# ChaitIITB/ReplicatingGPT

Measured on AMD Instinct MI355X. Metric: train tokens/sec at 1/2/4/8 MI355X + MFMA util, char-GPT block 256, higher is better.
Workload: dtype bf16; 1 GPU; c2: char-GPT 6L/6H/384d, block 256, batch 64/GPU, dropout 0.2, AdamW, full train step; global_batch=64, seq_len=256, parallelism=dp1, world_size=1, graph=True

## Files before the change

include/charpt.h:

```cpp
#ifndef CHARPT_H
#define CHARPT_H
#include <stdint.h>

#ifdef __cplusplus
extern "C" {
#endif

enum { CG_OK = 0, CG_EINVAL = 1, CG_EHIP = 2, CG_EUNSUPPORTED = 3 };
enum { CG_F32 = 0, CG_BF16 = 1 };
enum { CG_BITS = 2 };

enum {
    CG_EPI_STORE = 0,
    CG_EPI_BIAS = 1,
    CG_EPI_BIAS_RELU = 2,
    CG_EPI_BIAS_RESID = 3,
    CG_EPI_BIAS_DROP_RESID = 4,
    CG_EPI_RELU_BWD = 5,
    CG_EPI_STORE_ROWDOT = 7
};

typedef struct {
    int kind;
    const float* bias;
    const float* resid;
    int64_t ld_resid;
    const void* aux;
    int aux_dtype;
    int64_t ld_aux;
    double dropout_p;
    uint64_t seed;
    const uint64_t* rng_call;
    int site;
    float beta;
    float* colpart;
    int flags;
} cg_epilogue_t;

enum { CG_GEMM_SLAB_BF16 = 1, CG_GEMM_DEFER_REDUCE = 2 };
enum { CG_DEFER = 1 };

const char* cg_last_error_string(void);
int cg_version(void);
int cg_set_tuning(const char* key, int value);
int cg_device_info(int* n_cu, int* arch_major, int* arch_minor);
int cg_timing_event_create(void** event);
int cg_timing_event_record(void* event, void* stream);
int cg_timing_event_elapsed(void* start, void* end, float* ms);
int cg_timing_event_destroy(void* event);

int cg_counter_add(int64_t* counter, int64_t delta, void* stream);
int cg_rng_snapshot(uint64_t* counter, uint64_t* snap, void* stream);
int cg_dropout_mask(float* dst, int64_t n, double p, uint64_t seed, const uint64_t* rng_call, int site,
                    void* stream);
int cg_dropout_apply(const float* x, int64_t rows, int64_t C, int64_t ldx, void* y, int y_dtype, double p,
                     uint64_t seed, const uint64_t* rng_call, int site, void* stream);
int cg_sum_f32(const float* x, int64_t n, float scale, float* out, float* ws, void* stream);
int cg_cast_f32_bf16(const float* x, uint16_t* y, int64_t n, void* stream);

int cg_gather_batch(const void* data, int data_is_u8, const int64_t* ix, int64_t* x, int64_t* y,
                    int64_t B, int64_t T, void* stream);

int cg_gather_pairs(const int64_t* table, const int64_t* plen, const int64_t* tlen, const int64_t* ix, int64_t* x,
                    int64_t* y, int64_t B, int64_t T, int64_t pad_token, int64_t ignore_index, void* stream);

int cg_embed_fwd(const int64_t* idx, const float* wte, const float* wpe, float* x, int64_t B, int64_t T,
                 int64_t C, int64_t V, void* stream);
int64_t cg_embed_bwd_workspace(int64_t B, int64_t T, int64_t C, int64_t V);
int cg_embed_bwd(const int64_t* idx, const float* dx, float* dwte, float* dwpe, int64_t B, int64_t T,
                 int64_t C, int64_t V, int accumulate, void* workspace, void* stream);

int cg_layernorm_fwd(const float* x, const float* w, const float* b, void* y, int y_dtype, float* mean,
                     float* rstd, int64_t rows, int64_t C, float eps, void* stream);
int64_t cg_layernorm_bwd_workspace(int64_t rows, int64_t C);
int cg_layernorm_bwd(const void* dy, int dy_dtype, const float* x, const float* w, const float* mean,
                     const float* rstd, const float* dres, float* dx, uint16_t* dx_bf16, float* dw, float* db,
                     int accumulate, void* workspace, int64_t rows, int64_t C, void* stream);
int cg_layernorm_bwd_ex(const void* dy, int dy_dtype, const float* x, const float* w, const float* mean,
                        const float* rstd, const float* dres, float* dx, uint16_t* lp_out, double lp_dropout_p,
                        uint64_t lp_seed, const uint64_t* lp_rng_call, int lp_site, float* dw, float* db,
                        float* lp_colsum, int accumulate, int colsum_accumulate, void* workspace, int64_t rows,
                        int64_t C, void* stream);
int cg_layernorm_bwd_rows(const void* dy, int dy_dtype, const float* x, const float* w, const float* mean,
                          const float* rstd, const float* dres, float* dx, uint16_t* lp_out, double lp_dropout_p,
                          uint64_t lp_seed, const uint64_t* lp_rng_call, int lp_site, int lp_colsum,
                          void* workspace, int64_t rows, int64_t C, void* stream);
int cg_layernorm_bwd_reduce(const void* workspace, int64_t rows, int64_t C, int lp_colsum_partials, float* dw,
                            float* db, float* lp_colsum, int accumulate, int colsum_accumulate, void* stream);
int cg_layernorm_bwd_reduce_ex(const void* workspace, int64_t rows, int64_t C, int lp_colsum_partials, float* dw,
                               float* db, float* lp_colsum, int accumulate, int colsum_accumulate, int flags,
                               void* stream);

int64_t cg_gemm_workspace(int64_t M, int64_t N, int split_k);
int cg_gemm_colpart_supported(int a_trans, int b_trans, int64_t M, int64_t N, int64_t K, int64_t lda, int64_t ldb,
                              int64_t ldc);
int cg_gemm_relu_bits_supported(int a_trans, int b_trans, int64_t M, int64_t N, int64_t K, int64_t lda, int64_t ldb,
                                int64_t ldc);
// ... 145 lines not shown
```

replicatinggpt_amd/_lib.py:

```python
import ctypes
import os
import re

import torch

_HERE = os.path.dirname(os.path.abspath(__file__))
LIB_PATH = os.environ.get("CHARPT_LIB") or os.path.join(_HERE, "libcharpt_hip.so")
HEADER_PATH = os.path.join(os.path.dirname(_HERE), "include", "charpt.h")

CG_F32, CG_BF16, CG_BITS = 0, 1, 2
EPI_STORE, EPI_BIAS, EPI_BIAS_RELU, EPI_BIAS_RESID, EPI_BIAS_DROP_RESID, EPI_RELU_BWD = range(6)
EPI_STORE_ROWDOT = 7
GEMM_SLAB_BF16, GEMM_DEFER_REDUCE = 1, 2
DEFER = 1

c_i64, c_int, c_dbl, c_flt, c_u64, P = ctypes.c_int64, ctypes.c_int, ctypes.c_double, ctypes.c_float, ctypes.c_uint64, ctypes.c_void_p


class Epilogue(ctypes.Structure):
    _fields_ = [("kind", c_int), ("bias", P), ("resid", P), ("ld_resid", c_i64), ("aux", P), ("aux_dtype", c_int),
                ("ld_aux", c_i64), ("dropout_p", c_dbl), ("seed", c_u64), ("rng_call", P), ("site", c_int),
                ("beta", c_flt), ("colpart", P), ("flags", c_int)]


class WgradProblem(ctypes.Structure):
    _fields_ = [("M", c_i64), ("N", c_i64), ("K", c_i64), ("A", P), ("lda", c_i64), ("B", P), ("ldb", c_i64), ("C", P),
                ("ldc", c_i64), ("beta", c_flt), ("split_k", c_int), ("workspace", P), ("flags", c_int)]


_SIGS = {
    "cg_last_error_string": (ctypes.c_char_p, []),
    "cg_version": (c_int, []),
    "cg_set_tuning": (c_int, [ctypes.c_char_p, c_int]),
    "cg_device_info": (c_int, [P, P, P]),
    "cg_counter_add": (c_int, [P, c_i64, P]),
    "cg_rng_snapshot": (c_int, [P, P, P]),
    "cg_dropout_mask": (c_int, [P, c_i64, c_dbl, c_u64, P, c_int, P]),
    "cg_dropout_apply": (c_int, [P, c_i64, c_i64, c_i64, P, c_int, c_dbl, c_u64, P, c_int, P]),
    "cg_sum_f32": (c_int, [P, c_i64, c_flt, P, P, P]),
    "cg_cast_f32_bf16": (c_int, [P, P, c_i64, P]),
    "cg_gather_batch": (c_int, [P, c_int, P, P, P, c_i64, c_i64, P]),
    "cg_gather_pairs": (c_int, [P, P, P, P, P, P, c_i64, c_i64, c_i64, c_i64, P]),
    "cg_embed_fwd": (c_int, [P, P, P, P, c_i64, c_i64, c_i64, c_i64, P]),
    "cg_embed_bwd_workspace": (c_i64, [c_i64, c_i64, c_i64, c_i64]),
    "cg_embed_bwd": (c_int, [P, P, P, P, c_i64, c_i64, c_i64, c_i64, c_int, P, P]),
    "cg_layernorm_fwd": (c_int, [P, P, P, P, c_int, P, P, c_i64, c_i64, c_flt, P]),
    "cg_layernorm_bwd_workspace": (c_i64, [c_i64, c_i64]),
    "cg_layernorm_bwd": (c_int, [P, c_int, P, P, P, P, P, P, P, P, P, c_int, P, c_i64, c_i64, P]),
    "cg_layernorm_bwd_ex": (c_int, [P, c_int, P, P, P, P, P, P, P, c_dbl, c_u64, P, c_int, P, P, P, c_int, c_int, P,
                                    c_i64, c_i64, P]),
    "cg_layernorm_bwd_rows": (c_int, [P, c_int, P, P, P, P, P, P, P, c_dbl, c_u64, P, c_int, c_int, P, c_i64, c_i64,
                                      P]),
    "cg_layernorm_bwd_reduce": (c_int, [P, c_i64, c_i64, c_int, P, P, P, c_int, c_int, P]),
    "cg_layernorm_bwd_reduce_ex": (c_int, [P, c_i64, c_i64, c_int, P, P, P, c_int, c_int, c_int, P]),
    "cg_gemm_workspace": (c_i64, [c_i64, c_i64, c_int]),
    "cg_gemm_colpart_supported": (c_int, [c_int, c_int, c_i64, c_i64, c_i64, c_i64, c_i64, c_i64]),
    "cg_gemm_relu_bits_supported": (c_int, [c_int, c_int, c_i64, c_i64, c_i64, c_i64, c_i64, c_i64]),
    "cg_gemm_rowdot_supported": (c_int, [c_int, c_int, c_i64, c_i64, c_i64, c_i64, c_i64, c_i64]),
    "cg_linear_rows_f32_supported": (c_int, [c_i64, c_i64, c_i64]),
    "cg_decode_qkv_f32": (c_int, [c_i64, c_i64, c_i64, P, c_i64, P, P, c_flt, P, c_i64, P, c_i64, P, c_i64, P, P, P]),
    "cg_linear_rows_f32": (c_int, [c_i64, c_i64, c_i64, P, c_i64, P, P, c_flt, P, c_i64, P, c_int, P, c_i64, P, c_i64, P]),
    "cg_ffn_fwd_f32_supported": (c_int, [c_i64, c_i64, c_i64]),
    "cg_ffn_fwd_f32": (c_int, [c_i64, c_i64, c_i64, P, c_i64, P, P, c_flt, P, c_i64, P, P, c_i64, P, P, c_i64, P,
                               c_i64, P]),
    "cg_gemm_resid_layernorm_supported": (c_int, [c_i64, c_i64, c_i64]),
    "cg_gemm_resid_layernorm": (c_int, [c_i64, c_i64, c_i64, P, c_i64, P, c_i64, P, c_i64, ctypes.POINTER(Epilogue), P, P,
                                        P, P, P, c_flt, P]),
    "cg_flush_deferred": (c_int, [P]),
    "cg_discard_deferred": (c_int, [P, P]),
    "cg_reduce_rows": (c_int, [P, c_i64, c_i64, P, c_int, P]),
    "cg_reduce_rows_ex": (c_int, [P, c_i64, c_i64, P, c_int, c_int, P]),
    "cg_gemm": (c_int, [c_int, c_int, c_int, c_i64, c_i64, c_i64, P, c_i64, P, c_i64, P, c_int, c_i64,
                        ctypes.POINTER(Epilogue), c_int, P, P]),
    "cg_gemm_wgrad_group_supported": (c_int, [ctypes.POINTER(WgradProblem), c_int]),
    "cg_gemm_wgrad_group": (c_int, [ctypes.POINTER(WgradProblem), c_int, P]),
    "cg_colsum_workspace": (c_i64, [c_i64, c_i64]),
    "cg_colsum": (c_int, [P, c_int, c_i64, c_i64, c_i64, P, c_int, P, P]),
    "cg_attn_fwd": (c_int, [c_int, c_i64, c_i64, c_i64, c_i64, P, P, P, c_i64, P, c_i64, P, c_flt, c_dbl, c_u64, P,
                            c_int, P, P]),
    "cg_attn_fwd_premasked": (c_int, [c_int, c_i64, c_i64, c_i64, c_i64, P, P, P, c_i64, P, c_i64, P, c_flt, c_dbl,
                                      c_u64, P, c_int, P, P]),
    "cg_attn_dropmask": (c_int, [c_i64, c_i64, c_i64, c_dbl, c_u64, P, c_int, P, P]),
    "cg_layernorm_fwd_attn_dropmask": (c_int, [P, P, P, P, c_int, P, P, c_i64, c_i64, c_flt, c_i64, c_i64, c_i64,
                                               c_dbl, c_u64, P, c_int, P, P]),
    "cg_attn_mask_bytes": (c_i64, [c_i64, c_i64, c_i64]),
    "cg_attn_bwd_workspace": (c_i64, [c_i64, c_i64, c_i64, c_i64]),
    "cg_attn_bwd": (c_int, [c_int, c_i64, c_i64, c_i64, c_i64, P, P, P, c_i64, P, c_i64, P, c_i64, P, P, P, P, c_i64,
                            c_flt, c_dbl, c_u64, P, c_int, P, P, P]),
    "cg_attn_bwd_delta": (c_int, [c_int, c_i64, c_i64, c_i64, c_i64, P, P, P, c_i64, P, c_i64, P, c_i64, P, P, P, P,
                                  P, c_i64, c_flt, c_dbl, c_u64, P, c_int, P, P, P]),
    "cg_ce_fwd": (c_int, [P, c_i64, c_i64, c_i64, P, P, P, P]),
    "cg_ce_bwd": (c_int, [P, c_i64, c_i64, c_i64, P, P, P, c_flt, P, c_i64, P, P]),
    "cg_head_workspace": (c_i64, [c_i64, c_i64]),
    "cg_head_fwd": (c_int, [P, P, c_i64, P, P, P, P, P, P, c_i64, c_i64, c_i64, P]),
    "cg_head_bwd": (c_int, [P, P, P, P, c_flt, P, P, c_i64, P, c_int, P, c_i64, c_i64, P]),
    "cg_head_bwd_ex": (c_int, [P, P, P, P, c_flt, P, P, c_i64, P, c_int, P, c_i64, c_i64, c_int, P]),
    "cg_head_masked_workspace": (c_i64, [c_i64, c_i64]),
    "cg_head_fwd_masked": (c_int, [P, P, c_i64, P, P, c_i64, P, P, P, P, P, c_i64, c_i64, c_i64, P]),
    "cg_head_bwd_masked": (c_int, [P, P, P, c_i64, P, P, P, P, c_i64, P, c_int, P, c_i64, c_i64, c_int, P]),
    "cg_ce_fwd_masked": (c_int, [P, c_i64, c_i64, P, c_i64, P, P, P]),
    "cg_ce_mean_masked_workspace": (c_i64, [c_i64]),
    "cg_ce_mean_masked": (c_int, [P, P, c_i64, c_i64, P, P, P, P]),
    "cg_ce_bwd_masked": (c_int, [P, c_i64, c_i64, P, c_i64, P, P, P, P, P, P]),
    "cg_decode_window": (c_int, [P, c_i64, c_i64, c_i64, P, P, P]),
    "cg_decode_embed": (c_int, [P, c_i64, P, P, c_i64, P, P, c_i64, P]),
    "cg_decode_kv_append": (c_int, [P, c_i64, c_i64, c_i64, c_i64, c_i64, c_i64, c_i64, P, P, P, P]),
    "cg_decode_attn": (c_int, [P, c_i64, P, P, c_i64, c_i64, c_i64, c_i64, c_i64, c_i64, P, c_i64, c_flt, P, c_i64,
                               P]),
    "cg_decode_sample": (c_int, [P, c_i64, c_i64, c_i64, c_int, P, P, P, c_i64, P]),
    "cg_decode_sample_filtered": (c_int, [P, c_i64, c_i64, c_i64, P, P, P, P, c_i64, P]),
# ... 71 lines not shown
```

replicatinggpt_amd/csrc/gemm.hip:

```cpp
#include "defer.h"

using namespace cg;

namespace {

constexpr int GBM = 64, GBN = 64, GBK = 16;

template <typename TA, typename TB, typename TC>
__global__ __launch_bounds__(256) void k_gemm_generic(int a_trans, int b_trans, int64_t M, int64_t N, int64_t K,
                                                      const TA* __restrict__ A, int64_t lda,
                                                      const TB* __restrict__ B, int64_t ldb, TC* __restrict__ C,
                                                      int64_t ldc, EpiArgs epi, int split_k, int64_t kchunk,
                                                      float* __restrict__ ws) {
    __shared__ float As[GBK][GBM + 4];
    __shared__ float Bs[GBK][GBN + 4];
    const int tid = threadIdx.x, lane = tid & 63, wave = tid >> 6;
    const int wm = wave >> 1, wn = wave & 1;
    const int64_t tilesN = (N + GBN - 1) / GBN;
    const int64_t m0 = (int64_t)(blockIdx.x / tilesN) * GBM;
    const int64_t n0 = (int64_t)(blockIdx.x % tilesN) * GBN;
    const int split = blockIdx.y;
    const int64_t kb = split * kchunk;
    const int64_t ke = kb + kchunk < K ? kb + kchunk : K;

// ... 78 lines not shown
    a.ld_resid = e->ld_resid;
    a.aux = e->aux;
    a.aux_dtype = e->aux_dtype;
    a.ld_aux = e->ld_aux;
    a.thr = e->dropout_p > 0 ? dropout_threshold(e->dropout_p) : 0u;
    a.dscale = e->dropout_p > 0 ? dropout_scale(e->dropout_p) : 1.f;
    a.seed = e->seed;
    a.rng_call = e->rng_call;
    a.site = e->site;
    a.beta = e->beta;
    a.colpart = e->colpart;
    return a;
}

template <typename TA, typename TB>
int launch_generic(int a_trans, int b_trans, int64_t M, int64_t N, int64_t K, const void* A, int64_t lda,
                   const void* B, int64_t ldb, void* C, int c_dtype, int64_t ldc, const EpiArgs& e, int split_k,
                   void* ws, hipStream_t st) {
    int64_t kchunk = (K + split_k - 1) / split_k;
    kchunk = (kchunk + GBK - 1) / GBK * GBK;
    const int64_t tiles = ((M + GBM - 1) / GBM) * ((N + GBN - 1) / GBN);
    dim3 grid((unsigned)tiles, (unsigned)split_k);
    if (c_dtype == CG_BF16)
        k_gemm_generic<TA, TB, bf16_t><<<grid, 256, 0, st>>>(a_trans, b_trans, M, N, K, (const TA*)A, lda,
                                                             (const TB*)B, ldb, (bf16_t*)C, ldc, e, split_k, kchunk,
                                                             (float*)ws);
    else
        k_gemm_generic<TA, TB, float><<<grid, 256, 0, st>>>(a_trans, b_trans, M, N, K, (const TA*)A, lda,
                                                            (const TB*)B, ldb, (float*)C, ldc, e, split_k, kchunk,
                                                            (float*)ws);
    return CG_OK;
}

}

namespace cg {
int g_gemm_variant = 0;
int g_gemm_max_grid = 0;
int g_gemm_group_p8 = 0;
int g_gemm_group_pk = 0;
int g_gemm_n96 = 1;
}

extern "C" int cg_gemm_colpart_supported(int a_trans, int b_trans, int64_t M, int64_t N, int64_t K, int64_t lda,
                                         int64_t ldb, int64_t ldc) {
    return gemm_colpart_supported(a_trans, b_trans, M, N, K, lda, ldb, ldc) ? 1 : 0;
}

extern "C" int cg_gemm_relu_bits_supported(int a_trans, int b_trans, int64_t M, int64_t N, int64_t K, int64_t lda,
                                           int64_t ldb, int64_t ldc) {
    return gemm_relu_bits_supported(a_trans, b_trans, M, N, K, lda, ldb, ldc) ? 1 : 0;
}

extern "C" int cg_gemm_rowdot_supported(int a_trans, int b_trans, int64_t M, int64_t N, int64_t K, int64_t lda,
                                        int64_t ldb, int64_t ldc) {
    return gemm_rowdot_supported(a_trans, b_trans, M, N, K, lda, ldb, ldc) ? 1 : 0;
}

extern "C" int64_t cg_gemm_workspace(int64_t M, int64_t N, int split_k) {
    return split_k > 1 ? (int64_t)split_k * M * N * (int64_t)sizeof(float) : 0;
}

extern "C" int cg_gemm_resid_layernorm_supported(int64_t M, int64_t N, int64_t K) {
    return gemm_resid_ln_supported(M, N, K) ? 1 : 0;
}

extern "C" int cg_gemm_resid_layernorm(int64_t M, int64_t N, int64_t K, const void* A, int64_t lda, const void* W,
                                       int64_t ldw, float* out, int64_t ldc, const cg_epilogue_t* epi,
                                       const float* ln_w, const float* ln_b, void* y, float* mean, float* rstd,
                                       float eps, void* stream) {
    CG_REQUIRE(gemm_resid_ln_supported(M, N, K),
               "cg_gemm_resid_layernorm: unsupported shape M=%lld N=%lld K=%lld (N == 384, M %% 64 == 0, K %% 64 == 0)",
               (long long)M, (long long)N, (long long)K);
    CG_REQUIRE(epi && (epi->kind == CG_EPI_BIAS_RESID || epi->kind == CG_EPI_BIAS_DROP_RESID) && epi->bias &&
                   epi->resid && epi->beta == 0.f && epi->flags == 0 && !epi->colpart,
               "cg_gemm_resid_layernorm: needs a BIAS_RESID / BIAS_DROP_RESID epilogue with bias and residual, beta 0");
    CG_REQUIRE(A && W && out && ln_w && ln_b && y && mean && rstd, "cg_gemm_resid_layernorm: null pointer");
    CG_REQUIRE(lda >= K && ldw >= K && lda % 8 == 0 && ldw % 8 == 0 && ldc >= N && ldc % 4 == 0 &&
                   epi->ld_resid >= N && epi->ld_resid % 4 == 0,
               "cg_gemm_resid_layernorm: bad leading dimensions");
    CG_REQUIRE((((uintptr_t)A | (uintptr_t)W | (uintptr_t)out | (uintptr_t)epi->resid | (uintptr_t)epi->bias |
                 (uintptr_t)ln_w | (uintptr_t)ln_b | (uintptr_t)y) & 15) == 0,
               "cg_gemm_resid_layernorm: operands must be 16-B aligned");
    const EpiArgs e = make_epi(epi);
    gemm_resid_ln_launch(M, K, (const bf16_t*)A, lda, (const bf16_t*)W, ldw, out, ldc, e, ln_w, ln_b, (bf16_t*)y, mean,
                         rstd, eps, (hipStream_t)stream);
    CG_LAUNCH_CHECK("cg_gemm_resid_layernorm");
    return CG_OK;
}

extern "C" int cg_gemm(int op_dtype, int a_trans, int b_trans, int64_t M, int64_t N, int64_t K, const void* A,
                       int64_t lda, const void* B, int64_t ldb, void* C, int c_dtype, int64_t ldc,
                       const cg_epilogue_t* epi, int split_k, void* workspace, void* stream) {
    CG_REQUIRE(M > 0 && N > 0 && K > 0, "cg_gemm: empty problem M=%lld N=%lld K=%lld", (long long)M, (long long)N,
               (long long)K);
    CG_REQUIRE(split_k >= 1 && split_k <= 64, "cg_gemm: split_k out of range");
    CG_REQUIRE(split_k == 1 || workspace, "cg_gemm: split_k > 1 needs a workspace");
    CG_REQUIRE(op_dtype == CG_BF16 || op_dtype == CG_F32, "cg_gemm: bad op dtype");
    hipStream_t st = (hipStream_t)stream;
    EpiArgs e = make_epi(epi);
    CG_REQUIRE(split_k == 1 || e.kind == CG_EPI_STORE || e.kind == CG_EPI_BIAS || e.kind == CG_EPI_BIAS_RESID,
               "cg_gemm: split-K supports STORE/BIAS/BIAS_RESID epilogues only");
    const bool vec4 = N % 4 == 0 && ldc % 4 == 0 && M * N < (int64_t)1 << 31 &&
                      (((uintptr_t)C | (uintptr_t)workspace | (uintptr_t)(e.bias ? e.bias : (const float*)C) |
                        (uintptr_t)(e.resid ? e.resid : (const float*)C)) & 15) == 0 &&
                      (!e.resid || e.ld_resid % 4 == 0);
// ... 131 lines not shown
```

replicatinggpt_amd/csrc/gemm_bf16.hip:

```cpp
#include "gemm_tile.h"

namespace cg {
namespace {
using namespace gt;

template <bool TR, int R, int THREADS>
struct Operand {
    static constexpr int BYTES = R * FBK * 2;
    static constexpr int NCH = BYTES / (THREADS * 16);
    static_assert(NCH >= 1 && NCH * THREADS * 16 == BYTES, "tile/thread mismatch");
    struct Stage {
        uint4 v[NCH];
    };
    static __device__ __forceinline__ Stage load(const bf16_t* __restrict__ X, int64_t ld, int64_t r0, int64_t k0,
                                                 int tid) {
        Stage s;
#pragma unroll
        for (int i = 0; i < NCH; ++i) {
            const int lin = tid + i * THREADS;
            if (!TR) {
                const int r = lin >> 3, c = lin & 7;
                s.v[i] = *(const uint4*)(X + (r0 + r) * ld + k0 + c * 8);
            } else {
                constexpr int CPR = R / 8;
// ... 140 lines not shown
        v = (!at && split_k == 1 && M % 256 == 0 && N % 256 == 0 && t256 >= 2 * (int64_t)gemm_cu_count()) ? 24 : 9;
    }
    return v;
}

static bool fast_shape_ok(int64_t M, int64_t N, int64_t K, int64_t lda, int64_t ldb, int64_t ldc, int split_k) {
    return N % 128 == 0 && K % FBK == 0 && K / FBK >= split_k && M % 128 == 0 && lda % 8 == 0 && ldb % 8 == 0 &&
           ldc % 8 == 0;
}

#ifdef CG_AB_VARIANTS
static bool pk128(int v) { return v == 9 || v == 10 || v == 12; }
#else
static bool pk128(int v) { return v == 9; }
#endif

static bool colpart_ok(int v, int at, int split_k) {
    return (v == 24 || v == 26 || (pk128(v) && !(g_pk_flags & 2))) && split_k == 1 && !at;
}

bool gemm_colpart_supported(int at, int bt, int64_t M, int64_t N, int64_t K, int64_t lda, int64_t ldb, int64_t ldc) {
    return fast_shape_ok(M, N, K, lda, ldb, ldc, 1) && colpart_ok(pick_variant(at, bt, M, N, 1), at, 1);
}

static bool relu_bits_ok(int v, int at, int split_k, int64_t N) {
    return colpart_ok(v, at, split_k) && N % 64 == 0;
}

bool gemm_relu_bits_supported(int at, int bt, int64_t M, int64_t N, int64_t K, int64_t lda, int64_t ldb, int64_t ldc) {
    return fast_shape_ok(M, N, K, lda, ldb, ldc, 1) && relu_bits_ok(pick_variant(at, bt, M, N, 1), at, 1, N);
}

static bool rowdot_ok(int v, int at, int split_k, int64_t N) {
    return pk128(v) && !(g_pk_flags & 2) && split_k == 1 && !at && N % 64 == 0;
}

bool gemm_rowdot_supported(int at, int bt, int64_t M, int64_t N, int64_t K, int64_t lda, int64_t ldb, int64_t ldc) {
    return fast_shape_ok(M, N, K, lda, ldb, ldc, 1) && rowdot_ok(pick_variant(at, bt, M, N, 1), at, 1, N);
}

bool gemm_wgrad_group_ok(int64_t M, int64_t N, int64_t K, const void* A, int64_t lda, const void* B, int64_t ldb,
                         const void* C, int64_t ldc, int split_k) {
    if (split_k < 2 || !fast_shape_ok(M, N, K, lda, ldb, ldc, split_k)) return false;
    if ((((uintptr_t)A) | ((uintptr_t)B) | ((uintptr_t)C)) & 15) return false;
    if (pick_variant(1, 1, M, N, split_k) != 9) return false;
    const int64_t nkt = K / FBK, nkc = (nkt + split_k - 1) / split_k;
    if ((split_k - 1) * nkc >= nkt) return false;
    return M * N < ((int64_t)1 << 31) && K < ((int64_t)1 << 31);
}

bool fast_gemm_launch(int at, int bt, int64_t M, int64_t N, int64_t K, const bf16_t* A, int64_t lda, const bf16_t* B,
                      int64_t ldb, void* C, int c_dtype, int64_t ldc, const EpiArgs& e, int split_k, float* ws,
                      hipStream_t st) {
    if (!fast_shape_ok(M, N, K, lda, ldb, ldc, split_k)) return false;
    if ((((uintptr_t)A) | ((uintptr_t)B) | ((uintptr_t)C)) & 15) return false;
    if (e.bias && (((uintptr_t)e.bias) & 15)) return false;
    if (e.resid && ((((uintptr_t)e.resid) & 15) || e.ld_resid % 4)) return false;
    const bool aux_bits = e.aux_dtype == CG_BITS;
    if (e.aux && ((((uintptr_t)e.aux) & (aux_bits ? 7 : 15)) || e.ld_aux % (aux_bits ? 2 : 8))) return false;
    int v = pick_variant(at, bt, M, N, split_k);
    if (e.slab_bf16 && (!pk128(v) || split_k < 2 || e.kind != CG_EPI_STORE)) return false;
    if (K % (FBK * split_k)) {
        const int64_t nkt = K / FBK, nkc = (nkt + split_k - 1) / split_k;
        if (!pk128(v) || (split_k - 1) * nkc >= nkt) return false;
    }
    if (e.kind == CG_EPI_STORE_ROWDOT &&
        (!rowdot_ok(v, at, split_k, N) || !e.aux || e.aux_dtype != CG_BF16 || !e.colpart || e.ld_resid <= 0 ||
         M % e.ld_resid || e.beta != 0.f || c_dtype != CG_BF16 || (((uintptr_t)e.colpart) & 3)))
        return false;
    if (e.colpart && e.kind != CG_EPI_STORE_ROWDOT && (!colpart_ok(v, at, split_k) || e.kind != CG_EPI_RELU_BWD ||
                      (e.aux_dtype != CG_BF16 && e.aux_dtype != CG_BITS) || e.beta != 0.f || c_dtype != CG_BF16))
        return false;
    if (e.aux_dtype == CG_BITS &&
        (!relu_bits_ok(v, at, split_k, N) || (e.kind != CG_EPI_RELU_BWD && e.kind != CG_EPI_BIAS_RELU) ||
         (e.kind == CG_EPI_BIAS_RELU && !e.bias) || !e.aux || e.beta != 0.f || c_dtype != CG_BF16))
        return false;
    if (v >= 20 && p8_gemm_launch(v, at, bt, M, N, K, A, lda, B, ldb, C, c_dtype, ldc, e, split_k, ws, st))
        return true;
    if (e.aux_dtype == CG_BITS && !pk128(v)) return false;
    if (v >= 20) v = 2;
#ifdef CG_AB_VARIANTS
    if (v >= 5 && glds_gemm_launch(v, at, bt, M, N, K, A, lda, B, ldb, C, c_dtype, ldc, e, split_k, ws, st))
        return true;
#else
    if (v >= 5 && pk_gemm_launch(v, at, bt, M, N, K, A, lda, B, ldb, C, c_dtype, ldc, e, split_k, ws, st))
        return true;
#endif
#ifdef CG_AB_VARIANTS
    if ((v == 3 || v == 4) && M % 256) v = 1;
    switch (v) {
        case 3: launch<256, 128, 1>(at, bt, M, N, K, A, lda, B, ldb, C, c_dtype, ldc, e, split_k, ws, st); return true;
        case 4: launch<256, 128, 2>(at, bt, M, N, K, A, lda, B, ldb, C, c_dtype, ldc, e, split_k, ws, st); return true;
        case 1: launch<128, 128, 1>(at, bt, M, N, K, A, lda, B, ldb, C, c_dtype, ldc, e, split_k, ws, st); return true;
        default: break;
    }
#endif
    launch<128, 128, 2>(at, bt, M, N, K, A, lda, B, ldb, C, c_dtype, ldc, e, split_k, ws, st);
    return true;
}

}
```

replicatinggpt_amd/csrc/gemm_common.h:

```cpp
#pragma once
#include <type_traits>

#include "adamw.h"
#include "common.h"

namespace cg {

typedef float fv16f __attribute__((ext_vector_type(16)));

struct EpiArgs {
    int kind;
    const float* bias;
    const float* resid;
    int64_t ld_resid;
    const void* aux;
    int aux_dtype;
    int64_t ld_aux;
    uint32_t thr;
    float dscale;
    uint64_t seed;
    const uint64_t* rng_call;
    int site;
    float beta;
    float* colpart;
// ... 200 lines not shown
                        *(fv4*)(J.v + 4 * i) = vv[s];
                        *(uint2*)(J.pb + 4 * i) = make_uint2(pack_bf2(pv[s][0], pv[s][1]), pack_bf2(pv[s][2], pv[s][3]));
                    }
                }
            }
        }
        return;
    }
#endif
    for (int q = 0; q < r.na; ++q) {
        const AdamJob& J = r.a[q];
        const AdamScalars sc = adam_scalars(J.lr, J.beta1, J.beta2, J.eps, J.wd, J.step);
        for (int64_t i = t0; i < J.n4; i += nthr) {
            fv4 pv = *(const fv4*)(J.p + 4 * i);
            const fv4 gv = *(const fv4*)(J.g + 4 * i);
            fv4 mv = *(const fv4*)(J.m + 4 * i), vv = *(const fv4*)(J.v + 4 * i);
#pragma unroll
            for (int e = 0; e < 4; ++e) {
                float me = mv[e], ve = vv[e];
                pv[e] = adam_one(pv[e], gv[e], me, ve, sc);
                mv[e] = me;
                vv[e] = ve;
            }
            *(fv4*)(J.p + 4 * i) = pv;
            *(fv4*)(J.m + 4 * i) = mv;
            *(fv4*)(J.v + 4 * i) = vv;
            *(uint2*)(J.pb + 4 * i) = make_uint2(pack_bf2(pv[0], pv[1]), pack_bf2(pv[2], pv[3]));
        }
    }
}

extern int g_gemm_variant;
extern int g_gemm_max_grid;
extern int g_gemm_group_p8;
extern int g_gemm_group_pk;
extern int g_gemm_n96;
extern int g_linear_rows_nb;
extern int g_pk_flags;
int gemm_cu_count();

bool fast_gemm_launch(int at, int bt, int64_t M, int64_t N, int64_t K, const bf16_t* A, int64_t lda, const bf16_t* B,
                      int64_t ldb, void* C, int c_dtype, int64_t ldc, const EpiArgs& e, int split_k, float* ws,
                      hipStream_t st);
bool gemm_colpart_supported(int at, int bt, int64_t M, int64_t N, int64_t K, int64_t lda, int64_t ldb, int64_t ldc);
bool gemm_rowdot_supported(int at, int bt, int64_t M, int64_t N, int64_t K, int64_t lda, int64_t ldb, int64_t ldc);
bool gemm_relu_bits_supported(int at, int bt, int64_t M, int64_t N, int64_t K, int64_t lda, int64_t ldb, int64_t ldc);
bool glds_gemm_launch(int variant, int at, int bt, int64_t M, int64_t N, int64_t K, const bf16_t* A, int64_t lda,
                      const bf16_t* B, int64_t ldb, void* C, int c_dtype, int64_t ldc, const EpiArgs& e, int split_k,
                      float* ws, hipStream_t st);
bool pk_gemm_launch(int variant, int at, int bt, int64_t M, int64_t N, int64_t K, const bf16_t* A, int64_t lda,
                    const bf16_t* B, int64_t ldb, void* C, int c_dtype, int64_t ldc, const EpiArgs& e, int split_k,
                    float* ws, hipStream_t st);

constexpr int MAX_GROUP = 4;
struct GroupProb {
    const bf16_t* A;
    const bf16_t* B;
    void* ws;
    int64_t lda, ldb;
    int M, N;
    int tilesN, ntiles;
    int nkt, nkc;
    int split_k;
    int item0;
    int gm;
};
bool gemm_wgrad_group_ok(int64_t M, int64_t N, int64_t K, const void* A, int64_t lda, const void* B, int64_t ldb,
                         const void* C, int64_t ldc, int split_k);
void pk_group_launch(const GroupProb* probs, int n, bool slab_bf16, hipStream_t st);

bool gemm_resid_ln_supported(int64_t M, int64_t N, int64_t K);
void gemm_resid_ln_launch(int64_t M, int64_t K, const bf16_t* A, int64_t lda, const bf16_t* W, int64_t ldw, float* X,
                          int64_t ldx, const EpiArgs& e, const float* lnw, const float* lnb, bf16_t* Y, float* mean,
                          float* rstd, float eps, hipStream_t st);
bool p8_gemm_launch(int variant, int at, int bt, int64_t M, int64_t N, int64_t K, const bf16_t* A, int64_t lda,
                    const bf16_t* B, int64_t ldb, void* C, int c_dtype, int64_t ldc, const EpiArgs& e, int split_k,
                    float* ws, hipStream_t st);

}
```

replicatinggpt_amd/csrc/util.hip:

```cpp
#include <limits.h>
#include <stdarg.h>

#include "attention_common.h"
#include "defer.h"
#include "ln_fwd.h"

namespace cg {
static thread_local char g_err[1024] = "";
void set_error(const char* fmt, ...) {
    va_list ap;
    va_start(ap, fmt);
    vsnprintf(g_err, sizeof(g_err), fmt, ap);
    va_end(ap);
}
}

using namespace cg;

extern "C" const char* cg_last_error_string(void) { return g_err; }
extern "C" int cg_version(void) { return 1; }

extern "C" int cg_device_info(int* n_cu, int* major, int* minor) {
    int dev = 0;
    hipDeviceProp_t prop;
// ... 213 lines not shown
    size_t nd = 0;
    hipError_t r = hipStreamGetCaptureInfo_v2(st, &cs, &id, &g, &deps, &nd);
    if (r == hipSuccess && cs == hipStreamCaptureStatusActive) {
        hipGraphNode_t node = nullptr;
        r = hipGraphAddEventRecordNode(&node, g, deps, nd, (hipEvent_t)event);
        if (r == hipSuccess) r = hipStreamUpdateCaptureDependencies(st, &node, 1, hipStreamSetCaptureDependencies);
    } else if (r == hipSuccess) {
        r = hipEventRecord((hipEvent_t)event, st);
    }
    if (r != hipSuccess) {
        (void)hipGetLastError();
        cg::set_error("cg_timing_event_record: %s", hipGetErrorString(r));
        return CG_EHIP;
    }
    return CG_OK;
}

extern "C" int cg_timing_event_elapsed(void* start, void* end, float* ms) {
    CG_REQUIRE(start && end && ms, "cg_timing_event_elapsed: null");
    const hipError_t r = hipEventElapsedTime(ms, (hipEvent_t)start, (hipEvent_t)end);
    if (r != hipSuccess) {
        cg::set_error("cg_timing_event_elapsed: %s", hipGetErrorString(r));
        return CG_EHIP;
    }
    return CG_OK;
}

extern "C" int cg_timing_event_destroy(void* event) {
    if (event) (void)hipEventDestroy((hipEvent_t)event);
    return CG_OK;
}

namespace {
#ifdef CG_AB_VARIANTS
constexpr bool AB_BUILD = true;
#else
constexpr bool AB_BUILD = false;
#endif
constexpr int ANY_LO = INT_MIN, ANY_HI = INT_MAX;
constexpr int AB_LO(int lo) { return AB_BUILD ? ANY_LO : lo; }
constexpr int AB_HI(int hi) { return AB_BUILD ? ANY_HI : hi; }

struct Knob {
    const char* key;
    int* knob;
    int lo, hi;
};
const Knob KNOBS[] = {
    {"gemm_variant", &g_gemm_variant, ANY_LO, ANY_HI},
    {"gemm_max_grid", &g_gemm_max_grid, ANY_LO, ANY_HI},
    {"gemm_group_p8", &g_gemm_group_p8, 0, 255},
    {"gemm_group_pk", &g_gemm_group_pk, 0, 255},
    {"gemm_n96", &g_gemm_n96, ANY_LO, ANY_HI},
    {"pk_flags", &g_pk_flags, ANY_LO, ANY_HI},
    {"linear_rows_nb", &g_linear_rows_nb, 0, 2},
    {"skip_splitk_reduce", &g_skip_splitk_reduce, ANY_LO, ANY_HI},
    {"adam_per_launch", &g_adam_per_launch, ANY_LO, ANY_HI},
    {"adam_batch", &g_adam_batch, AB_LO(1), AB_HI(1)},
    {"red_side", &g_red_side, ANY_LO, ANY_HI},
    {"attn_variant", &g_attn_variant, AB_LO(0), AB_HI(2)},
    {"attn_bwd_lpt", &g_attn_bwd_lpt, 0, 1},
    {"decode_attn_rows", &g_decode_attn_rows, 0, 1},
    {"adamw_mode", &g_adamw_mode, 0, 5},
    {"ln_rl", &g_ln_rl, 0, 2},
    {"ln_nt", &g_ln_nt, ANY_LO, ANY_HI},
    {"ln_pf", &g_ln_pf, ANY_LO, ANY_HI},
    {"ln_waves", &g_ln_waves, ANY_LO, ANY_HI},
    {"ln_rpb", &g_ln_rpb, ANY_LO, ANY_HI},
};

bool gemm_variant_in_product(int v) {
    return v == 0 || v == 2 || v == 9 || v == 24 || v == 96 || v == 97 || v == 98 || v == 99;
}
}

extern "C" int cg_set_tuning(const char* key, int value) {
    CG_REQUIRE(key, "cg_set_tuning: null key");
    if (!strcmp(key, "defer_splitk") || !strcmp(key, "slab_bf16") || !strcmp(key, "defer_partials")) {
        set_error("cg_set_tuning: %s is a per-call flag since round 5 (cg_epilogue_t.flags CG_GEMM_DEFER_REDUCE / "
                  "CG_GEMM_SLAB_BF16, the CG_DEFER flag of the _ex reduces)", key);
        return CG_EINVAL;
    }
    for (const Knob& k : KNOBS) {
        if (strcmp(key, k.key)) continue;
        const bool ok = value >= k.lo && value <= k.hi &&
                        (AB_BUILD || k.knob != &g_gemm_variant || gemm_variant_in_product(value));
        CG_REQUIRE(ok, "cg_set_tuning: %s = %d is not accepted by this build (out of range, or an A/B variant: make ab)",
                   key, value);
        *k.knob = value;
        return CG_OK;
    }
    set_error("cg_set_tuning: unknown key %s", key);
    return CG_EINVAL;
}
```

Baseline: 5.856 million tokens/s.

## Add persistent B-stationary GEMM kernel for wide-N MLP shapes

Adds a persistent GEMM kernel in which each block keeps one 128-column panel of B in registers and streams 64-row tiles of A through a triple-buffered LDS pipeline. It runs by default for large-M, N>=1152 GEMMs with K<=384 and store, bias-ReLU, or ReLU-backward epilogues; in this model those are the MLP up-projection and its gradient. The ReLU epilogue also writes the sign bitmask, and the backward epilogue applies that mask and can emit column partial sums. The aim is to avoid reloading the weight panel for every output tile and to overlap A loads with MFMA work. The cost is one block per CU and heavy register use, so latency hiding may suffer.

Measured after the change: 5.986 million tokens/s (median of 6 runs). 1.02x the previous value.

```diff
diff --git a/include/charpt.h b/include/charpt.h
--- a/include/charpt.h
+++ b/include/charpt.h
@@ -43,6 +43,7 @@
 const char* cg_last_error_string(void);
 int cg_version(void);
 int cg_set_tuning(const char* key, int value);
+int64_t cg_gemm_ws_launches(void);
 int cg_device_info(int* n_cu, int* arch_major, int* arch_minor);
 int cg_timing_event_create(void** event);
 int cg_timing_event_record(void* event, void* stream);
diff --git a/replicatinggpt_amd/_lib.py b/replicatinggpt_amd/_lib.py
--- a/replicatinggpt_amd/_lib.py
+++ b/replicatinggpt_amd/_lib.py
@@ -56,6 +56,7 @@
     "cg_gemm_workspace": (c_i64, [c_i64, c_i64, c_int]),
     "cg_gemm_colpart_supported": (c_int, [c_int, c_int, c_i64, c_i64, c_i64, c_i64, c_i64, c_i64]),
     "cg_gemm_relu_bits_supported": (c_int, [c_int, c_int, c_i64, c_i64, c_i64, c_i64, c_i64, c_i64]),
+    "cg_gemm_ws_launches": (c_i64, []),
     "cg_gemm_rowdot_supported": (c_int, [c_int, c_int, c_i64, c_i64, c_i64, c_i64, c_i64, c_i64]),
     "cg_linear_rows_f32_supported": (c_int, [c_i64, c_i64, c_i64]),
     "cg_decode_qkv_f32": (c_int, [c_i64, c_i64, c_i64, P, c_i64, P, P, c_flt, P, c_i64, P, c_i64, P, c_i64, P, P, P]),
diff --git a/replicatinggpt_amd/csrc/gemm.hip b/replicatinggpt_amd/csrc/gemm.hip
--- a/replicatinggpt_amd/csrc/gemm.hip
+++ b/replicatinggpt_amd/csrc/gemm.hip
@@ -154,6 +154,8 @@
     return gemm_relu_bits_supported(a_trans, b_trans, M, N, K, lda, ldb, ldc) ? 1 : 0;
 }
 
+extern "C" int64_t cg_gemm_ws_launches(void) { return (int64_t)ws_gemm_launches(); }
+
 extern "C" int cg_gemm_rowdot_supported(int a_trans, int b_trans, int64_t M, int64_t N, int64_t K, int64_t lda,
                                         int64_t ldb, int64_t ldc) {
     return gemm_rowdot_supported(a_trans, b_trans, M, N, K, lda, ldb, ldc) ? 1 : 0;
diff --git a/replicatinggpt_amd/csrc/gemm_bf16.hip b/replicatinggpt_amd/csrc/gemm_bf16.hip
--- a/replicatinggpt_amd/csrc/gemm_bf16.hip
+++ b/replicatinggpt_amd/csrc/gemm_bf16.hip
@@ -216,6 +216,11 @@
 bool fast_gemm_launch(int at, int bt, int64_t M, int64_t N, int64_t K, const bf16_t* A, int64_t lda, const bf16_t* B,
                       int64_t ldb, void* C, int c_dtype, int64_t ldc, const EpiArgs& e, int split_k, float* ws,
                       hipStream_t st) {
+    if (g_gemm_variant == 31 ||
+        (g_gemm_variant == 0 && ws_gemm_auto(M, N, e.kind) && fast_shape_ok(M, N, K, lda, ldb, ldc, split_k) &&
+         pick_variant(at, bt, M, N, split_k) == 9)) {
+        if (ws_gemm_launch(at, bt, M, N, K, A, lda, B, ldb, C, c_dtype, ldc, e, split_k, st)) return true;
+    }
     if (!fast_shape_ok(M, N, K, lda, ldb, ldc, split_k)) return false;
     if ((((uintptr_t)A) | ((uintptr_t)B) | ((uintptr_t)C)) & 15) return false;
     if (e.bias && (((uintptr_t)e.bias) & 15)) return false;
diff --git a/replicatinggpt_amd/csrc/gemm_common.h b/replicatinggpt_amd/csrc/gemm_common.h
--- a/replicatinggpt_amd/csrc/gemm_common.h
+++ b/replicatinggpt_amd/csrc/gemm_common.h
@@ -276,6 +276,12 @@
                     const bf16_t* B, int64_t ldb, void* C, int c_dtype, int64_t ldc, const EpiArgs& e, int split_k,
                     float* ws, hipStream_t st);
 
+extern int g_gemm_ws;
+bool ws_gemm_auto(int64_t M, int64_t N, int kind);
+bool ws_gemm_launch(int at, int bt, int64_t M, int64_t N, int64_t K, const bf16_t* A, int64_t lda, const bf16_t* B,
+                    int64_t ldb, void* C, int c_dtype, int64_t ldc, const EpiArgs& e, int split_k, hipStream_t st);
+long long ws_gemm_launches();
+
 constexpr int MAX_GROUP = 4;
 struct GroupProb {
     const bf16_t* A;
diff --git a/replicatinggpt_amd/csrc/gemm_ws.hip b/replicatinggpt_amd/csrc/gemm_ws.hip
--- /dev/null
+++ b/replicatinggpt_amd/csrc/gemm_ws.hip
@@ -0,0 +1,303 @@
+#include "gemm_pk.h"
+
+namespace cg {
+int g_gemm_ws = 1;
+namespace {
+using namespace gt;
+
+long long g_ws_launches = 0;
+
+constexpr int WS_NBUF = 3;
+constexpr int WS_KT_A = 64 * 64 * 2;
+constexpr int WS_KT_B = 64 * 128 * 2;
+constexpr int WS_XCHG = 8 * 1024;
+constexpr int WS_BITS = 1024;
+constexpr int WS_LPT = 1;
+constexpr int WS_STORES = 2;
+
+constexpr int ws_lds_bytes(int nkt) { return WS_NBUF * nkt * WS_KT_A + WS_XCHG + WS_NBUF * WS_BITS; }
+
+__device__ __forceinline__ void store_pair(uint32_t x0, uint32_t y0, uint32_t x1, uint32_t y1, bf16_t* C, int64_t ldc,
+                                           int64_t m, int64_t nb, int q) {
+    const int64_t col = nb + ((q & 1) ? 16 : 0) + ((q >> 1) ? 8 : 0);
+    const auto sx = __builtin_amdgcn_permlane16_swap(x0, x1, false, false);
+    const auto sy = __builtin_amdgcn_permlane16_swap(y0, y1, false, false);
+    st_out16((uint4*)(C + m * ldc + col), make_uint4(sx[0], sy[0], sx[1], sy[1]));
+}
+
+__device__ __forceinline__ float bf_lo(uint32_t w) { return __uint_as_float(w << 16); }
+__device__ __forceinline__ float bf_hi(uint32_t w) { return __uint_as_float(w & 0xffff0000u); }
+
+template <bool BT, int EK, int NKT>
+__global__ __launch_bounds__(512, 1) __attribute__((amdgpu_waves_per_eu(1, 2)))
+void k_gemm_ws(int M, int N, const bf16_t* __restrict__ A, int64_t lda, const bf16_t* __restrict__ B, int64_t ldb,
+               bf16_t* __restrict__ C, int64_t ldc, const float* __restrict__ bias, uint32_t* __restrict__ bits,
+               int64_t ldw, float* __restrict__ colpart) {
+    static_assert(NKT >= 1 && NKT <= 6, "K <= 384");
+    constexpr int STAGE = NKT * WS_KT_A;
+    static_assert(!BT || NKT * WS_KT_B <= (WS_NBUF - 1) * STAGE, "the transposed panel fits in stages 1..");
+    extern __shared__ __attribute__((aligned(16))) char smem[];
+    const int tid = threadIdx.x, lane = tid & 63, wave = __builtin_amdgcn_readfirstlane(tid >> 6);
+    const int wr = wave >> 2, wc = wave & 3, g = lane >> 4;
+    const int npanels = N / 128, P = gridDim.x, bpp = P / npanels;
+    const int lb = xcd_remap(blockIdx.x, P);
+    const int panel = lb % npanels, rslot = lb / npanels;
+    if (rslot >= bpp) return;
+    const int T = M / 64, base = T / bpp, rem = T % bpp;
+    const int ntile = base + (rslot < rem ? 1 : 0);
+    if (ntile == 0) return;
+    const int tile0 = rslot * base + (rslot < rem ? rslot : rem);
+    const int64_t n0 = (int64_t)panel * 128, nb = n0 + wc * 32;
+
+    const uint32_t lds0 = lds_base(smem);
+    char* const xchg = smem + WS_NBUF * STAGE;
+    const uint32_t bits0 = lds0 + (uint32_t)(WS_NBUF * STAGE + WS_XCHG);
+    DmaP<false, 64, 8, FBK> da;
+    da.init(lda, wave, lane);
+    auto issue_a = [&](int t, int kt, int sg) {
+        const bf16_t* src = A + (int64_t)(tile0 + t) * 64 * lda + kt * FBK;
+        da.issue1(src, 0, lds0 + (uint32_t)(sg * STAGE + kt * WS_KT_A), wave);
+    };
+    const uint32_t bits_off = (uint32_t)(lane * (int)ldw * 4);
+    auto issue_bits = [&](int t, int sg) {
+        if (EK == CG_EPI_RELU_BWD && wave == 0)
+            dma16sl(bits + (int64_t)(tile0 + t) * 64 * ldw + panel * 4, bits_off, bits0 + (uint32_t)(sg * WS_BITS));
+    };
+
+    issue_bits(0, 0);
+#pragma unroll
+    for (int kt = 0; kt < NKT; ++kt) issue_a(0, kt, 0);
+    sv8 bw[NKT][2][2];
+    if constexpr (!BT) {
+#pragma unroll
+        for (int kt = 0; kt < NKT; ++kt)
+#pragma unroll
+            for (int s = 0; s < 2; ++s)
+#pragma unroll
+                for (int j = 0; j < 2; ++j)
+                    bw[kt][s][j] = *(const sv8*)(B + (nb + 16 * j + (lane & 15)) * ldb + kt * FBK + 32 * s + 8 * g);
+    } else {
+        DmaP<true, 128, 8, FBK> db;
+        db.init(ldb, wave, lane);
+#pragma unroll
+        for (int kt = 0; kt < NKT; ++kt)
+#pragma unroll
+            for (int i = 0; i < 2; ++i)
+                db.issue1(B + (int64_t)kt * FBK * ldb + n0, i, lds0 + (uint32_t)(STAGE + kt * WS_KT_B), wave);
+        wait_vm<0>();
+        __builtin_amdgcn_s_barrier();
+#pragma unroll
+        for (int kt = 0; kt < NKT; ++kt)
+#pragma unroll
+            for (int s = 0; s < 2; ++s)
+#pragma unroll
+                for (int j = 0; j < 2; ++j)
+                    bw[kt][s][j] = frag<true, 128>(smem + STAGE + kt * WS_KT_B, wc * 32 + 16 * j, s, lane);
+        asm volatile("s_waitcnt lgkmcnt(0)" ::: "memory");
+        __builtin_amdgcn_s_barrier();
+    }
+    float4 bv[2];
+    if constexpr (EK == CG_EPI_BIAS_RELU) {
+#pragma unroll
+        for (int j = 0; j < 2; ++j) bv[j] = *(const float4*)(bias + nb + 4 * g + 16 * j);
+    }
+    if (ntile > 1) {
+        issue_bits(1, 1);
+#pragma unroll
+        for (int kt = 0; kt < NKT; ++kt) issue_a(1, kt, 1);
+    }
+
+    constexpr int LPT = NKT * WS_LPT;
+    int sg = 0;
+    for (int t = 0; t < ntile; ++t) {
+        const bool more = t + 1 < ntile;
+        if (t > 0) {
+            if (more) wait_vm<LPT + WS_STORES>();
+            else wait_vm<WS_STORES>();
+        } else {
+            if (more) wait_vm<LPT>();
+            else wait_vm<0>();
+        }
+        asm volatile("s_waitcnt lgkmcnt(0)" ::: "memory");
+        __builtin_amdgcn_s_barrier();
+        const bool pf = t + 2 < ntile;
+        const int sg2 = sg == 0 ? 2 : sg - 1;
+        const char* img = smem + sg * STAGE;
+        if (pf) issue_bits(t + 2, sg2);
+
+        fv4 acc[2][2];
+#pragma unroll
+        for (int i = 0; i < 2; ++i)
+#pragma unroll
+            for (int j = 0; j < 2; ++j) acc[i][j] = fv4{0.f, 0.f, 0.f, 0.f};
+        sv8 af[2][2][2];
+        auto read_a = [&](int kt) {
+#pragma unroll
+            for (int s = 0; s < 2; ++s)
+#pragma unroll
+                for (int i = 0; i < 2; ++i)
+                    af[kt & 1][s][i] = frag<false, 64>(img + kt * WS_KT_A, wr * 32 + 16 * i, s, lane);
+        };
+        read_a(0);
+#pragma unroll
+        for (int kt = 0; kt < NKT; ++kt) {
+            if (kt + 1 < NKT) read_a(kt + 1);
+#pragma unroll
+            for (int s = 0; s < 2; ++s)
+#pragma unroll
+                for (int i = 0; i < 2; ++i)
+#pragma unroll
+                    for (int j = 0; j < 2; ++j) acc[i][j] = mfma_bf16(bw[kt][s][j], af[kt & 1][s][i], acc[i][j]);
+            if (pf) issue_a(t + 2, kt, sg2);
+        }
+
+        const int64_t mr = (int64_t)(tile0 + t) * 64 + wr * 32 + (lane & 15);
+        uint32_t px[2][2], py[2][2];
+        if constexpr (EK == CG_EPI_BIAS_RELU) {
+            uint32_t w[2];
+#pragma unroll
+            for (int i = 0; i < 2; ++i) {
+#pragma unroll
+                for (int j = 0; j < 2; ++j) {
+                    fv4& v = acc[i][j];
+                    v[0] = fmaxf(v[0] + bv[j].x, 0.f); v[1] = fmaxf(v[1] + bv[j].y, 0.f);
+                    v[2] = fmaxf(v[2] + bv[j].z, 0.f); v[3] = fmaxf(v[3] + bv[j].w, 0.f);
+                    px[i][j] = pack_bf2(v[0], v[1]);
+                    py[i][j] = pack_bf2(v[2], v[3]);
+                }
+                w[i] = (nz4_bf16(make_uint2(px[i][0], py[i][0])) << (4 * g)) |
+                       (nz4_bf16(make_uint2(px[i][1], py[i][1])) << (16 + 4 * g));
+                w[i] |= (uint32_t)__shfl_xor((int)w[i], 16, 64);
+                w[i] |= (uint32_t)__shfl_xor((int)w[i], 32, 64);
+            }
+            if (bits && g < 2) bits[(mr + 16 * g) * ldw + (nb >> 5)] = g ? w[1] : w[0];
+        } else if constexpr (EK == CG_EPI_RELU_BWD) {
+            const char* bimg = smem + WS_NBUF * STAGE + WS_XCHG + sg * WS_BITS;
+#pragma unroll
+            for (int i = 0; i < 2; ++i) {
+                const uint32_t w = *(const uint32_t*)(bimg + (wr * 32 + 16 * i + (lane & 15)) * 16 + wc * 4);
+#pragma unroll
+                for (int j = 0; j < 2; ++j) {
+                    const uint32_t kb = (w >> (16 * j + 4 * g)) & 0xfu;
+                    fv4& v = acc[i][j];
+#pragma unroll
+                    for (int q = 0; q < 4; ++q) v[q] = ((kb >> q) & 1u) ? v[q] : 0.f;
+                    px[i][j] = pack_bf2(v[0], v[1]);
+                    py[i][j] = pack_bf2(v[2], v[3]);
+                }
+            }
+            if (colpart) {
+                uint4* xp = (uint4*)(xchg + (wc * 64 + lane) * 32);
+                if (wr == 1) {
+                    xp[0] = make_uint4(px[0][0], py[0][0], px[0][1], py[0][1]);
+                    xp[1] = make_uint4(px[1][0], py[1][0], px[1][1], py[1][1]);
+                }
+                asm volatile("s_waitcnt lgkmcnt(0)" ::: "memory");
+                __builtin_amdgcn_s_barrier();
+                if (wr == 0) {
+                    const uint4 o2 = xp[0], o3 = xp[1];
+                    const uint32_t u2[2][2] = {{o2.x, o2.y}, {o2.z, o2.w}}, u3[2][2] = {{o3.x, o3.y}, {o3.z, o3.w}};
+                    float* cp = colpart + (int64_t)(tile0 + t) * N + nb + 4 * g;
+#pragma unroll
+                    for (int j = 0; j < 2; ++j) {
+                        fv4 s;
+                        s[0] = ((bf_lo(px[0][j]) + bf_lo(px[1][j])) + bf_lo(u2[j][0])) + bf_lo(u3[j][0]);
+                        s[1] = ((bf_hi(px[0][j]) + bf_hi(px[1][j])) + bf_hi(u2[j][0])) + bf_hi(u3[j][0]);
+                        s[2] = ((bf_lo(py[0][j]) + bf_lo(py[1][j])) + bf_lo(u2[j][1])) + bf_lo(u3[j][1]);
+                        s[3] = ((bf_hi(py[0][j]) + bf_hi(py[1][j])) + bf_hi(u2[j][1])) + bf_hi(u3[j][1]);
+                        fv4 r;
+#pragma unroll
+                        for (int q = 0; q < 4; ++q) r[q] = row16_sum_dpp(s[q]);
+                        if ((lane & 15) == 0) *(fv4*)(cp + 16 * j) = r;
+                    }
+                }
+                __builtin_amdgcn_sched_barrier(0);
+            }
+        } else {
+#pragma unroll
+            for (int i = 0; i < 2; ++i)
+#pragma unroll
+                for (int j = 0; j < 2; ++j) {
+                    px[i][j] = pack_bf2(acc[i][j][0], acc[i][j][1]);
+                    py[i][j] = pack_bf2(acc[i][j][2], acc[i][j][3]);
+                }
+        }
+#pragma unroll
+        for (int i = 0; i < 2; ++i) store_pair(px[i][0], py[i][0], px[i][1], py[i][1], C, ldc, mr + 16 * i, nb, g);
+        sg = sg == WS_NBUF - 1 ? 0 : sg + 1;
+    }
+    wait_vm<0>();
+}
+
+template <bool BT, int EK>
+void launch_nkt(int nkt, unsigned grid, int M, int N, const bf16_t* A, int64_t lda, const bf16_t* B, int64_t ldb,
+                bf16_t* C, int64_t ldc, const float* bias, uint32_t* bits, int64_t ldw, float* colpart, hipStream_t st) {
+#define WS(NKT_)                                                                                                   \
+    case NKT_:                                                                                                     \
+        k_gemm_ws<BT, EK, NKT_><<<grid, 512, ws_lds_bytes(NKT_), st>>>(M, N, A, lda, B, ldb, C, ldc, bias, bits, ldw, \
+                                                                      colpart);                                    \
+        break
+    switch (nkt) {
+        WS(1); WS(2); WS(3); WS(4); WS(5); WS(6);
+        default: break;
+    }
+#undef WS
+}
+
+}
+
+long long ws_gemm_launches() { return g_ws_launches; }
+
+bool ws_gemm_auto(int64_t M, int64_t N, int kind) {
+    const int only = g_gemm_ws == 2 ? CG_EPI_STORE : g_gemm_ws == 3 ? CG_EPI_BIAS_RELU : g_gemm_ws == 4 ? CG_EPI_RELU_BWD : -1;
+    return g_gemm_ws && (only < 0 || kind == only) && N >= 1152 && M >= 4096;
+}
+
+bool ws_gemm_launch(int at, int bt, int64_t M, int64_t N, int64_t K, const bf16_t* A, int64_t lda, const bf16_t* B,
+                    int64_t ldb, void* C, int c_dtype, int64_t ldc, const EpiArgs& e, int split_k, hipStream_t st) {
+    if (at || split_k != 1 || e.beta != 0.f || c_dtype != CG_BF16 || g_pk_flags) return false;
+    if (K % FBK || K > 6 * FBK || M % 64 || N % 128 || lda % 8 || ldb % 8 || ldc % 8) return false;
+    if (M >= ((int64_t)1 << 31) || N >= ((int64_t)1 << 31)) return false;
+    if (lda >= ((int64_t)1 << 24) || ldb >= ((int64_t)1 << 24)) return false;
+    if ((((uintptr_t)A) | ((uintptr_t)B) | ((uintptr_t)C)) & 15) return false;
+    const bool with_bits = e.aux_dtype == CG_BITS && e.aux;
+    uint32_t* bits = with_bits ? (uint32_t*)e.aux : nullptr;
+    switch (e.kind) {
+        case CG_EPI_STORE:
+            if (e.colpart) return false;
+            break;
+        case CG_EPI_BIAS_RELU:
+            if (!e.bias || (((uintptr_t)e.bias) & 15) || e.colpart) return false;
+            if (e.aux_dtype == CG_BITS && (!e.aux || (((uintptr_t)e.aux) & 3) || e.ld_aux < N / 32)) return false;
+            break;
+        case CG_EPI_RELU_BWD:
+            if (!with_bits || (((uintptr_t)e.aux) & 15) || e.ld_aux % 4 || e.ld_aux < N / 32 ||
+                e.ld_aux >= ((int64_t)1 << 24))
+                return false;
+            if (e.colpart && (((uintptr_t)e.colpart) & 15)) return false;
+            break;
+        default: return false;
+    }
+    int64_t P = gemm_cu_count();
+    if (g_gemm_max_grid > 0 && g_gemm_max_grid < P) P = g_gemm_max_grid;
+    if (P < N / 128) return false;
+    const int nkt = (int)(K / FBK);
+#define WSL(BT_, EK_)                                                                                               \
+    launch_nkt<BT_, EK_>(nkt, (unsigned)P, (int)M, (int)N, A, lda, B, ldb, (bf16_t*)C, ldc, e.bias, bits, e.ld_aux, \
+                         e.colpart, st)
+    if (e.kind == CG_EPI_STORE) {
+        if (bt) WSL(true, CG_EPI_STORE);
+        else WSL(false, CG_EPI_STORE);
+    } else if (e.kind == CG_EPI_BIAS_RELU) {
+        if (bt) WSL(true, CG_EPI_BIAS_RELU);
+        else WSL(false, CG_EPI_BIAS_RELU);
+    } else {
+        if (bt) WSL(true, CG_EPI_RELU_BWD);
+        else WSL(false, CG_EPI_RELU_BWD);
+    }
+#undef WSL
+    ++g_ws_launches;
+    return true;
+}
+
+}
diff --git a/replicatinggpt_amd/csrc/util.hip b/replicatinggpt_amd/csrc/util.hip
--- a/replicatinggpt_amd/csrc/util.hip
+++ b/replicatinggpt_amd/csrc/util.hip
@@ -289,6 +289,7 @@
     {"gemm_group_p8", &g_gemm_group_p8, 0, 255},
     {"gemm_group_pk", &g_gemm_group_pk, 0, 255},
     {"gemm_n96", &g_gemm_n96, ANY_LO, ANY_HI},
+    {"gemm_ws", &g_gemm_ws, 0, 4},
     {"pk_flags", &g_pk_flags, ANY_LO, ANY_HI},
     {"linear_rows_nb", &g_linear_rows_nb, 0, 2},
     {"skip_splitk_reduce", &g_skip_splitk_reduce, ANY_LO, ANY_HI},
@@ -307,7 +308,7 @@
 };
 
 bool gemm_variant_in_product(int v) {
-    return v == 0 || v == 2 || v == 9 || v == 24 || v == 96 || v == 97 || v == 98 || v == 99;
+    return v == 0 || v == 2 || v == 9 || v == 24 || v == 31 || v == 96 || v == 97 || v == 98 || v == 99;
 }
 }
 
```
